# klory/vqa-attention-networks

Measured on AMD Instinct MI355X. Metric: QA-pairs/sec fwd+bwd, MFB-baseline batch 512, higher is better.
Workload: dtype f32

## Files before the change

### include/vqa_fusion.h

```cpp
#ifndef VQA_FUSION_H
#define VQA_FUSION_H

#include <stddef.h>
#include <stdint.h>

#ifdef __cplusplus
extern "C" {
#endif

#define VQF_OK 0
#define VQF_E_BADARG (-1)
#define VQF_E_ALIGN (-2)
#define VQF_E_UNSUPPORTED (-3)
#define VQF_E_WORKSPACE (-4)
#define VQF_E_TIMEOUT (-5)

#define VQF_POOL_K 5

#define VQF_GEMM_RELU 1
#define VQF_GEMM_ACCUM 2
#define VQF_GEMM_OUT_BF16 4

int vqf_abi_version(void);
const char* vqf_build_info(void);
// ... 4 lines not shown
#define VQF_OPT_GEMM_BF16_LOOP 3
#define VQF_OPT_GEMM_F32_BIG 4
#define VQF_OPT_GEMM_BF16_BIG 5
#define VQF_OPT_GEMM_F32_WAVE 6
#define VQF_OPT_FUSE_COAL 7
#define VQF_OPT_FUSE_LS 8
#define VQF_OPT_FUSE_LS_BWD 9
#define VQF_OPT_GEMM_CU_LIMIT 10
#define VQF_OPT_GEMM_F32_EDGE 11
#define VQF_OPT_GEMM_F32_ROUNDS 12
#define VQF_OPT_GEMM_SPLITK_FUSED 13
#define VQF_OPT_GEMM_F32_STREAMK 14
#define VQF_OPT_GEMM_SPLITK_ORDER 15
#define VQF_OPT_GEMM_F32_SAMPLE 16
#define VQF_OPT_GEMM_F32_N80 17
#define VQF_OPT_COUNT 18
int vqf_set_option(int option, int value, int* previous);
int vqf_get_option(int option, int* value);
const char* vqf_option_env_name(int option);

#define VQF_STAT_GEMM_F32_TILE128 0
#define VQF_STAT_GEMM_F32_BIG 1
#define VQF_STAT_GEMM_F32_WAVE 2
#define VQF_STAT_GEMM_BF16_TILE128 3
#define VQF_STAT_GEMM_BF16_BIG 4
#define VQF_STAT_GEMM_F32_SAMPLE 5
#define VQF_STAT_GEMM_F32_N80 6
#define VQF_STAT_COUNT 7
int vqf_stat_get(int stat, long long* value);

size_t vqf_gemm_f32_ws_bytes(int ta, int tb, int M, int N, int K);
int vqf_gemm_f32(int ta, int tb, int M, int N, int K,
                 const float* A, int lda, const float* B, int ldb,
                 float* C, int ldc, const float* bias, int flags,
                 void* ws, size_t ws_bytes, void* stream);

int vqf_gemm_f32_rowscale(int ta, int tb, int M, int N, int K, const float* A, int lda, const float* B, int ldb,
                          float* C, int ldc, const float* bias, int flags, const float* rowscale, int rows_per_scale,
                          void* stream);

int vqf_gemm_f32_big_rows(int ta, int tb, int M, int N, int K);
int vqf_gemm_f32_sample_supported(int NS, int L, int N, int K);
int vqf_gemm_f32_sample(int tb, int NS, int L, int N, int K, const float* A, int lda, const float* B, int ldb, float* C, int ldc,
// ... 261 lines not shown
int vqf_lstm_seq_supported(int B, int H);
size_t vqf_lstm_seq_ws_bytes(int B, int H);
#define VQF_LSTM_BF16 1
int vqf_lstm_seq_fwd(const float* xw, const float* w_hh, int S, int B, int H,
                     float* hs, float* cs, float* gates, int flags, void* ws, size_t ws_bytes, void* stream);
int vqf_lstm_seq_bwd(const float* dhs, const float* gates, const float* cs, const float* w_hh,
                     int S, int B, int H, float* dgates, float* dc_carry, int flags, void* ws, size_t ws_bytes,
                     void* stream);

int vqf_lstm_cell_fwd(float* gates, const float* c_prev, int B, int H, float* c_out, float* h_out, void* stream);
int vqf_lstm_step_supported(int B, int H);
int vqf_lstm_step_fwd(const float* h_prev, const float* w_hh, float* gates, const float* c_prev, int B, int H,
                      float* c_out, float* h_out, void* stream);
int vqf_lstm_cell_bwd(const float* dhs_t, const float* dh_carry, const float* gates, const float* c_t,
                      const float* c_prev, int first, int B, int H, float* dc_carry, float* dG, void* stream);

int vqf_embed_tanh_fwd(const float* W, const long long* ids, int T, int V, int E, float* out, void* stream);
int vqf_embed_tanh_bwd(const float* dout, const float* out, const long long* ids, int T, int V, int E, float* dW,
                       void* stream);
int vqf_embed_fwd(const float* W, const long long* ids, int T, int V, int E, float* out, void* stream);
int vqf_embed_bwd(const float* dout, const long long* ids, int T, int V, int E, float* dW, void* stream);
int vqf_embed_dropout_fwd(const float* W, const long long* ids, int T, int V, int E, const uint8_t* keep, uint64_t seed, float p_drop,
                          float* out, void* stream);
int vqf_embed_dropout_bwd(const float* dout, const long long* ids, int T, int V, int E, const uint8_t* keep, uint64_t seed, float p_drop,
                          float* dW, void* stream);
int vqf_embed_tanh_fwd_tm(const float* W, const long long* ids, int N, int Tq, int V, int E, float* out, void* stream);
int vqf_embed_tanh_bwd_tm(const float* dout, const float* out, const long long* ids, int N, int Tq, int V, int E, float* dW,
                          void* stream);

int vqf_feat_transpose(const float* src, int N, int D, int L, int out_bf16, void* dst, void* stream);
// ... 46 lines not shown
```

### vqa-attention-networks_amd/csrc/common.h

```cpp
#pragma once
#include <hip/hip_runtime.h>
#include <stdint.h>
#include "../../include/vqa_fusion.h"

typedef float f32x4 __attribute__((ext_vector_type(4)));
typedef float f32x16 __attribute__((ext_vector_type(16)));
typedef unsigned int u32x4 __attribute__((ext_vector_type(4)));

enum VqfKernelId {
  KID_GEMM_A0B0 = 0,
  KID_GEMM_A0B1,
  KID_GEMM_A1B0,
  KID_GEMM_A1B1,
  KID_SPLITK_REDUCE,
  KID_COLSUM,
  KID_GROUP_REDUCE,
  KID_RELU_BWD,
  KID_ATT_LOGITS_FWD,
  KID_ATT_LOGITS_BWD,
  KID_GLIMPSE_FWD,
  KID_GLIMPSE_BWD,
  KID_MFB_FUSE_FWD,
  KID_L2_GROUP_NORM,
  KID_SCALE_ROWS,
// ... 28 lines not shown
  KID_HIE_SLABSUM,
  KID_HIE_AFF,
  KID_PHRASE_FWD,
  KID_PHRASE_BWD,
  KID_HIE_AFF_LEVELS,
  KID_GUIDED_FWD,
  KID_GUIDED_BWD,
  KID_CE_LOSS_PRED,
  KID_ANSWER_MATCH,
  KID_TOPK_ROWS,
  KID_GLIMPSE_DFEAT_GROUPED,
  KID_ROW_BLOCK_GATHER,
  KID_ROW_BLOCK_GROUP_SUM,
  KID_MFB_FUSE_BWD_IMAGE,
  KID_ZERO_COLS,
  KID_COUNT
};

extern int g_vqf_prof_on;
extern int g_vqf_opt[VQF_OPT_COUNT];
static inline int vqf_opt(int id, int dflt) { const int v = g_vqf_opt[id]; return v < 0 ? dflt : v; }
extern long long g_vqf_stat[VQF_STAT_COUNT];
static inline void vqf_stat_bump(int id) { __atomic_fetch_add(&g_vqf_stat[id], 1LL, __ATOMIC_RELAXED); }
bool vqf_prof_begin(int id, hipStream_t s);
void vqf_prof_end(int id, hipStream_t s);
void vqf_prof_dims(int d0, int d1, int d2);

#define VQF_LAUNCH(id, kern, grid, block, shmem, stream, ...)                      \
  do {                                                                             \
    (void)hipGetLastError();     \
// ... 11 lines not shown
int* vqf_splitk_counters(int tiles);

int vqf_gemm_bf16_big_try(int ta, int tb, int M, int N, int K, const void* A, int lda, const void* B, int ldb, float* C,
                          int ldc, const float* bias, int flags, const float* rowscale, int rps, void* ws, size_t ws_bytes,
                          hipStream_t s, int* rc);
size_t vqf_gemm_bf16_big_ws_bytes(int ta, int tb, int M, int N, int K);
int vqf_gemm_f32_big_try(int ta, int tb, int M, int N, int K, const float* A, int lda, const float* B, int ldb, float* C,
                         int ldc, const float* bias, int flags, const float* rowscale, int rps, void* ws, size_t ws_bytes,
                         hipStream_t s, int* rc, int* rows_done);
int vqf_gemm_f32_big_rows_impl(int ta, int tb, int M, int N, int K, int flags, size_t ws_bytes);
size_t vqf_gemm_f32_big_ws_bytes(int ta, int tb, int M, int N, int K);
int vqf_gemm_f32_n80_try(int M, int N, int K, const float* A, int lda, const float* B, int ldb, float* C, int ldc,
                         const float* bias, int flags, hipStream_t s, int* rc);
int vqf_lstm_step16_try(const float* h_prev, const float* w_hh, float* gates, const float* c_prev, int B, int H, float* c_out,
                        float* h_out, hipStream_t s, int* rc);
int vqf_gemm_f32_wave_try(int ta, int tb, int M, int N, int K, const float* A, int lda, const float* B, int ldb, float* C,
                          int ldc, const float* bias, int flags, hipStream_t s, int* rc);

static inline int vqf_last_error() {
  hipError_t e = hipGetLastError();
  return e == hipSuccess ? VQF_OK : (int)e;
}

static inline bool aligned16(const void* p) { return (((uintptr_t)p) & 15) == 0; }

struct VqfDynLdsFlags { int bytes[64]; };
static inline int vqf_set_dyn_lds(const void* fn, int bytes, VqfDynLdsFlags& f) {
  int dev = 0;
  (void)hipGetDevice(&dev);
  const bool tracked = dev >= 0 && dev < 64;
// ... 187 lines not shown
```

### vqa-attention-networks_amd/csrc/gemm_f32_n80.hip

```cpp
#include "common.h"

namespace {

typedef const float __attribute__((address_space(1))) gfloat;

constexpr int TM = 128, TN = 80, TK = 32, NT = 512, NSLOT = 4;
constexpr int A_BYTES = TM * TK * 4;
constexpr int b_bytes(int ntc) { return 16 * ntc * TK * 4; }
constexpr int slot_bytes(int ntc) { return A_BYTES + b_bytes(ntc); }

struct N80Args {
  const float* A; const float* B; float* C; const float* bias;
  int M, N, K, lda, ldb, ldc, flags, tiles_m, tiles;
  const float* c_prev; float* c_out; float* h_out; int H;
};

__device__ __forceinline__ float sigm_f(float x) { return 1.0f / (1.0f + expf(-x)); }

__device__ __forceinline__ int swz(int rho) {
  const int i = (rho >> 1) & 7;
  return i ^ (((i + 2) & 4) >> 1);
}

__device__ __forceinline__ void wait_own(int later, bool two) {
// ... 136 lines not shown
#pragma unroll
  for (int t = 0; t < NTC; ++t) {
    const int col = n0 + 16 * t + c;
    if (col < g.N) {
      const float bv = g.bias ? g.bias[col] : 0.f;
#pragma unroll
      for (int j = 0; j < 4; ++j) {
        const int row = m0 + 16 * wave + 4 * kq + j;
        if (row < g.M) {
          float v = acc[t][j] + bv;
          if (relu) v = fmaxf(v, 0.f);
          g.C[(long long)row * g.ldc + col] = v;
        }
      }
    }
  }
}

}

int vqf_gemm_f32_n80_try(int M, int N, int K, const float* A, int lda, const float* B, int ldb, float* C, int ldc,
                         const float* bias, int flags, hipStream_t s, int* rc) {
  if (vqf_opt(VQF_OPT_GEMM_F32_N80, 1) == 0) return 0;
  if ((flags & ~VQF_GEMM_RELU) || (K % 128) || K < 512 || !aligned16(A) || !aligned16(B) || (lda % 4) || (ldb % 4)) return 0;
  const int tiles_m = (M + TM - 1) / TM, tiles_n = (N + TN - 1) / TN;
  const long long tiles = (long long)tiles_m * tiles_n;
  const int cus = vqf_cu_count() > 0 ? vqf_cu_count() : 256;
  if (tiles > cus || tiles * 10 < (long long)cus * 8 || M > 1024) return 0;
  if (vqf_opt(VQF_OPT_GEMM_CU_LIMIT, 0) >= 8) return 0;
  N80Args g;
// ... 18 lines not shown
  const int cus = vqf_cu_count() > 0 ? vqf_cu_count() : 256;
  if (tiles > cus || tiles * 10 < (long long)cus * 8) return 0;
  N80Args g = {};
  g.A = h_prev; g.B = w_hh; g.C = gates; g.M = B; g.N = 4 * H; g.K = H; g.lda = H; g.ldb = H; g.ldc = 4 * H;
  g.tiles_m = tiles_m; g.tiles = (int)tiles;
  g.c_prev = c_prev; g.c_out = c_out; g.h_out = h_out; g.H = H;
  const int nwg = ((int)tiles + 7) & ~7;
  vqf_prof_dims(B, 4 * H, H);
  vqf_stat_bump(VQF_STAT_GEMM_F32_N80);
  static VqfDynLdsFlags attr = {};
  if (int e = vqf_set_dyn_lds(reinterpret_cast<const void*>(&gemm_f32_n80_kernel<4, true>), NSLOT * slot_bytes(4), attr)) { *rc = e; return 1; }
  VQF_LAUNCH(KID_LSTM_CELL_FWD, (gemm_f32_n80_kernel<4, true>), dim3(nwg), dim3(NT), NSLOT * slot_bytes(4), s, g);
  *rc = vqf_last_error();
  return 1;
}
```

### vqa-attention-networks_amd/csrc/gemm_f32_wave.hip

```cpp
#include "common.h"
#include <stdlib.h>

namespace {

typedef const float __attribute__((address_space(1))) gfloat;
typedef float f32x2 __attribute__((ext_vector_type(2)));

constexpr int WTM = 32, WTN = 64, TK = 16, NSLOT = 6, NT = 256;
constexpr int A_BYTES = WTM * TK * 4, B_BYTES = WTN * TK * 4, SLOT_BYTES = A_BYTES + B_BYTES;
constexpr int WAVE_LDS = NSLOT * SLOT_BYTES;
constexpr int SMEM_WAVE = 4 * WAVE_LDS;
constexpr int NGA = A_BYTES / 1024, NGB = B_BYTES / 1024, NGL = NGA + NGB;

struct WaveArgs {
  const float* A;
  const float* B;
  float* C;
  const float* bias;
  int M, N, K, lda, ldb, ldc, flags;
  int tiles_m, tiles_n, kpart;
  const float* c_prev;
  float* c_out;
  float* h_out;
  int H;
};

__device__ __forceinline__ int swz(int r) { return (r >> 2) & 3; }

template <bool TB>
__device__ __forceinline__ void init_src(gfloat* (&q)[NGL], const WaveArgs& g, int m0, int n0, int k0, int lane) {
#pragma unroll
  for (int i = 0; i < NGA; ++i) {
    const int row = 16 * i + (lane >> 2);
    const int chunk = (lane & 3) ^ swz(row);
    q[i] = (gfloat*)(g.A + (long long)min(m0 + row, g.M - 1) * g.lda + k0 + chunk * 4);
  }
#pragma unroll
  for (int i = 0; i < NGB; ++i) {
    if (!TB) {
// ... 61 lines not shown

__device__ __forceinline__ void c_prefetch(const WaveArgs& g, int m0, int n0, int lane, bool vec, f32x2 (&cold)[16]) {
  const int cm = lane & 31, h = lane >> 5, col = n0 + 2 * cm;
#pragma unroll
  for (int e = 0; e < 16; ++e) {
    cold[e] = f32x2{0.f, 0.f};
    const int row = m0 + (e & 3) + 8 * (e >> 2) + 4 * h;
    if ((g.flags & VQF_GEMM_ACCUM) && row < g.M && col < g.N) {
      const float* pc = g.C + (long long)row * g.ldc + col;
      if (vec && col + 1 < g.N) cold[e] = *reinterpret_cast<const f32x2*>(pc);
      else { cold[e][0] = pc[0]; if (col + 1 < g.N) cold[e][1] = pc[1]; }
    }
  }
}

template <bool TB, int WK>
__global__ void __launch_bounds__(NT, 1) gemm_f32_wave_kernel(const WaveArgs g) {
  extern __shared__ __attribute__((aligned(16))) char smem[];
  const int tid = threadIdx.x, lane = tid & 63;
  const int wave = __builtin_amdgcn_readfirstlane(tid >> 6);
  const int nwg = gridDim.x, bid = blockIdx.x;
  const int q8 = nwg >> 3, r8 = nwg & 7, xcd = bid & 7;
  const int wg = (xcd < r8 ? xcd * (q8 + 1) : r8 * (q8 + 1) + (xcd - r8) * q8) + (bid >> 3);
  const int t = (WK == 1) ? 4 * wg + wave : wg;
  const int ntiles = g.tiles_m * g.tiles_n;
  const bool live = t < ntiles;
  const int tm = live ? t % g.tiles_m : 0, tn = live ? t / g.tiles_m : 0;
  const int m0 = tm * WTM, n0 = tn * WTN;
  const int k0 = (WK == 1) ? 0 : wave * g.kpart;
  const int S = live ? g.kpart / TK : 0;
  char* my = smem + wave * WAVE_LDS;

  f32x16 acc[2];
#pragma unroll
  for (int j = 0; j < 2; ++j)
#pragma unroll
    for (int e = 0; e < 16; ++e) acc[j][e] = 0.f;

  gfloat* q[NGL];
  init_src<TB>(q, g, m0, n0, k0, lane);
#pragma unroll
  for (int p = 0; p < NSLOT - 1; ++p)
    if (p < S) stage<TB>(q, g, my + p * SLOT_BYTES);
  const bool vec = ((g.ldc & 1) == 0) && ((reinterpret_cast<uintptr_t>(g.C) & 7) == 0);
  f32x2 cold[16];
  if (WK == 1 && live) c_prefetch(g, m0, n0, lane, vec, cold);
  Frag<TB> fa[2], fb[2];
  int slot = 0;
  auto half = [&](int s, Frag<TB> (&cur)[2], Frag<TB> (&nxt)[2]) {
    const bool more = s + 1 < S, refill = s + NSLOT - 1 < S;
    if (more) wait_copies(min(NSLOT - 3, S - 2 - s));
    const char* nx = my + (slot + 1 == NSLOT ? 0 : slot + 1) * SLOT_BYTES;
    char* rf = my + ((slot == 0) ? NSLOT - 1 : slot - 1) * SLOT_BYTES;
    typedef __attribute__((address_space(3))) char lds_char;
#pragma unroll
    for (int n = 0; n < 16; ++n) {
      const int ks = n >> 3, e = (n >> 1) & 3, j = n & 1;
      acc[j] = __builtin_amdgcn_mfma_f32_32x32x2f32(cur[ks].a[e], cur[ks].b(j, e), acc[j], 0, 0, 0);
      if (n == 0 && more) nxt[0].load(nx, 0, lane);
      if (n == 2 && more) nxt[1].load(nx, 1, lane);
      if (n >= 4 && n < 4 + NGL && refill) {
// ... 19 lines not shown
    half(s, fa, fb);
    if (s + 1 < S) half(s + 1, fb, fa);
  }

  const int cm = lane & 31, h = lane >> 5;
  if (WK == 1) {
    if (!live) return;
    const int col = n0 + 2 * cm;
    const float b0 = (g.bias && col < g.N) ? g.bias[col] : 0.f;
    const float b1 = (g.bias && col + 1 < g.N) ? g.bias[col + 1] : 0.f;
#pragma unroll
    for (int e = 0; e < 16; ++e)
      put2(g, m0 + (e & 3) + 8 * (e >> 2) + 4 * h, col, acc[0][e], acc[1][e], b0, b1, vec, cold[e][0], cold[e][1]);
  } else {
    asm volatile("s_waitcnt vmcnt(0)" ::: "memory");
    f32x2* mine = reinterpret_cast<f32x2*>(my);
#pragma unroll
    for (int e = 0; e < 16; ++e) mine[e * 64 + lane] = f32x2{acc[0][e], acc[1][e]};
    __syncthreads();
    if (!live) return;
    const int col = n0 + 2 * cm;
    const float b0 = (g.bias && col < g.N) ? g.bias[col] : 0.f;
    const float b1 = (g.bias && col + 1 < g.N) ? g.bias[col + 1] : 0.f;
#pragma unroll
    for (int qd = 0; qd < 4; ++qd) {
      const int e = wave + 4 * qd;
      f32x2 v = reinterpret_cast<const f32x2*>(smem)[e * 64 + lane];
#pragma unroll
      for (int w = 1; w < 4; ++w) {
        const f32x2 p = reinterpret_cast<const f32x2*>(smem + w * WAVE_LDS)[e * 64 + lane];
        v[0] += p[0]; v[1] += p[1];
      }
      float c0 = 0.f, c1 = 0.f;
      const int row = m0 + (e & 3) + 8 * (e >> 2) + 4 * h;
      if ((g.flags & VQF_GEMM_ACCUM) && row < g.M && col < g.N) {
        c0 = g.C[(long long)row * g.ldc + col];
        if (col + 1 < g.N) c1 = g.C[(long long)row * g.ldc + col + 1];
      }
      put2(g, row, col, v[0], v[1], b0, b1, vec, c0, c1);
    }
  }
}

constexpr int NGS = NGA + 1;

__device__ __forceinline__ void wait_copies3(int later) {
  switch (later < 0 ? 0 : later) {
    case 0:  asm volatile("s_waitcnt vmcnt(0)" ::: "memory"); break;
    case 1:  asm volatile("s_waitcnt vmcnt(3)" ::: "memory"); break;
// ... 245 lines not shown
    pc[2 * H] = a1;
    const float f_act = __shfl_xor(a0, 16, 64), o_act = __shfl_xor(a1, 16, 64);
    if (lo) {
      const float c = f_act * cpv[e] + a0 * a1;
      g.c_out[(long long)row * H + u0 + cm] = c;
      g.h_out[(long long)row * H + u0 + cm] = o_act * tanhf(c);
    }
  }
}

int launch_lstm_fwd(const WaveArgs& g, int nwg, hipStream_t s) {
  static VqfDynLdsFlags attr = {};
  constexpr int SMEM_SHB = 6 * (4 * A_BYTES + B_BYTES);
  if (int e = vqf_set_dyn_lds(reinterpret_cast<const void*>(&gemm_f32_lstm_fwd_kernel), SMEM_SHB, attr)) return e;
  VQF_LAUNCH(KID_LSTM_CELL_FWD, gemm_f32_lstm_fwd_kernel, dim3(nwg), dim3(NT), SMEM_SHB, s, g);
  return vqf_last_error();
}

template <bool TB, int WK>
int launch(const WaveArgs& g, int nwg, hipStream_t s) {
  static VqfDynLdsFlags attr = {};
  if (int e = vqf_set_dyn_lds(reinterpret_cast<const void*>(&gemm_f32_wave_kernel<TB, WK>), SMEM_WAVE, attr)) return e;
  VQF_LAUNCH(KID_GEMM_A0B0 + (TB ? 1 : 0), (gemm_f32_wave_kernel<TB, WK>), dim3(nwg), dim3(NT), SMEM_WAVE, s, g);
  return vqf_last_error();
}

}

int vqf_gemm_f32_wave_try(int ta, int tb, int M, int N, int K, const float* A, int lda, const float* B, int ldb, float* C,
                          int ldc, const float* bias, int flags, hipStream_t s, int* rc) {
// ... 38 lines not shown
  {
    int rc = VQF_OK;
    if (vqf_lstm_step16_try(h_prev, w_hh, gates, c_prev, B, H, c_out, h_out, (hipStream_t)stream, &rc)) return rc;
  }
  WaveArgs g = {};
  g.A = h_prev; g.B = w_hh; g.C = gates; g.bias = nullptr;
  g.M = B; g.N = 4 * H; g.K = H; g.lda = H; g.ldb = H; g.ldc = 4 * H; g.flags = VQF_GEMM_ACCUM;
  g.tiles_m = B / WTM;
  g.tiles_n = H / 16;
  g.kpart = H;
  g.c_prev = c_prev; g.c_out = c_out; g.h_out = h_out; g.H = H;
  vqf_prof_dims(B, 4 * H, H);
  vqf_stat_bump(VQF_STAT_GEMM_F32_WAVE);
  return launch_lstm_fwd(g, g.tiles_m * g.tiles_n / 4, (hipStream_t)stream);
}
```

### vqa-attention-networks_amd/csrc/prof.hip

```cpp
#include "common.h"
#include <mutex>
#include <stdlib.h>
#include <vector>

int g_vqf_prof_on = 0;
int g_vqf_opt[VQF_OPT_COUNT];
long long g_vqf_stat[VQF_STAT_COUNT] = {};

namespace {
const char* const kOptEnv[VQF_OPT_COUNT] = {
    "VQF_GEMM_F32_PERSIST", "VQF_GEMM_BF16_PERSIST", "VQF_GEMM_F32_LOOP", "VQF_GEMM_BF16_LOOP", "VQF_GEMM_F32_BIG",
    "VQF_GEMM_BF16_BIG", "VQF_GEMM_F32_WAVE", "VQF_FUSE_COAL", "VQF_FUSE_LS", "VQF_FUSE_LS_BWD", "VQF_GEMM_CU_LIMIT",
    "VQF_GEMM_F32_EDGE", "VQF_GEMM_F32_ROUNDS", "VQF_GEMM_SPLITK_FUSED", "VQF_GEMM_F32_STREAMK", "VQF_GEMM_SPLITK_ORDER", "VQF_GEMM_F32_SAMPLE", "VQF_GEMM_F32_N80"};
const char* const kOptEnvOld[VQF_OPT_COUNT] = {
    nullptr, nullptr, "VQF_GEMM_F32_PP", "VQF_GEMM_BF16_PP", nullptr, nullptr, nullptr, nullptr, nullptr, nullptr, nullptr,
    nullptr, nullptr, nullptr, nullptr, nullptr, nullptr};
struct OptInit {
  OptInit() {
    for (int i = 0; i < VQF_OPT_COUNT; ++i) {
      const char* e = getenv(kOptEnv[i]);
      if (!e && kOptEnvOld[i]) e = getenv(kOptEnvOld[i]);
      g_vqf_opt[i] = (e && ((e[0] >= '0' && e[0] <= '9') || e[0] == '-')) ? atoi(e) : -1;
    }
  }
} g_opt_init;
}

namespace {
// ... 5 lines not shown
thread_local int t_dims[3] = {0, 0, 0};
long long g_min_mnk = 0;

const char* const kNames[KID_COUNT] = {
    "gemm_f32_a0b0(fwd)", "gemm_f32_a0b1(dgrad)", "gemm_f32_a1b0", "gemm_f32_a1b1(wgrad)",
    "splitk_reduce", "colsum", "group_reduce", "relu_bwd",
    "att_logits_fwd", "att_logits_bwd", "glimpse_pool_fwd", "glimpse_pool_bwd",
    "mfb_fuse_fwd", "l2_group_norm", "scale_rows", "rowdot", "l2_norm_bwd_coef", "mfb_fuse_bwd",
    "dropout", "tanh_dropout_fwd", "tanh_dropout_bwd", "softmax_rows_fwd", "softmax_rows_bwd",
    "gemm_bf16", "cast_f32_bf16",
    "lstm_seq_fwd(all steps)", "lstm_seq_bwd(all steps)",
    "ce_loss", "kldiv_loss", "adam_step", "feat_transpose",
    "lstm_cell_fwd", "lstm_cell_bwd", "embed_tanh_fwd", "embed_tanh_bwd", "hbm_copy", "hbm_read_sweep", "multi_add", "multi_copy", "hie_hv_fwd", "hie_head_bwd", "hie_rank_add", "hie_rank_left", "hie_slab_sum", "hie_affinity",
    "phrase_ngram_fwd", "phrase_ngram_bwd", "hie_affinity_levels", "guided_logits_fwd", "guided_logits_bwd",
    "ce_loss_pred", "answer_match_rows", "topk_rows", "glimpse_dfeat_grouped", "row_block_gather", "row_block_group_sum",
    "mfb_fuse_bwd_image", "zero_cols_len"};

hipEvent_t get_event() {
  std::lock_guard<std::mutex> lk(g_mu);
  if (!g_free.empty()) { hipEvent_t e = g_free.back(); g_free.pop_back(); return e; }
  hipEvent_t e = nullptr;
  (void)hipEventCreate(&e);
  return e;
}
}

bool vqf_prof_begin(int id, hipStream_t s) {
  if (g_min_mnk > 0) {
    const bool gemm = (id >= KID_GEMM_A0B0 && id <= KID_GEMM_A1B1) || id == KID_GEMM_BF16;
    if (!gemm || (long long)t_dims[0] * t_dims[1] * t_dims[2] < g_min_mnk) return false;
  }
// ... 70 lines not shown
```

### vqa-attention-networks_amd/host/functions.py

```python
import torch

from . import ops


def _c(t):
    return t if t.is_contiguous() else t.contiguous()


def _w2d(w):
    return _c(w.reshape(w.shape[0], -1))


def _bf16_ok(*dims):
    return all(d % 8 == 0 for d in dims)


class EmbedTanhFn(torch.autograd.Function):

    @staticmethod
    def forward(ctx, ids, weight, tanh=True, time_major=False, lens=None):
        ids = ids.contiguous()
        out = ops.embed_tanh_fwd(_c(weight), ids, tanh, time_major, lens=lens)
        ctx.save_for_backward(ids, out if tanh else None)
        ctx.V, ctx.tm, ctx.lens = weight.shape[0], bool(time_major), lens
# ... 1005 lines not shown
                    ops.gemm(hs[t - 1], whh, out=gates[t], accumulate=True)
            ops.lstm_cell_fwd(gates[t], cs[t - 1] if t else None, cs[t], hs[t])
        ctx.save_for_backward(x, w_ih, w_hh, hs, cs, gates, xb, wb)
        ctx.has_bias = b_ih is not None
        return hs

    @staticmethod
    def backward(ctx, dhs):
        x, w_ih, w_hh, hs, cs, gates, xb, wb = ctx.saved_tensors
        T, B, I = x.shape
        H = w_hh.shape[1]
        dhs = _c(dhs)
        whh = ops.cast_bf16(_c(w_hh)) if ctx.bf16 else _c(w_hh)
        dG = torch.empty_like(gates)
        dc = torch.empty((B, H), dtype=torch.float32, device=x.device)
        dh = None
        for t in range(T - 1, -1, -1):
            ops.lstm_cell_bwd(dhs[t], dh, gates[t], cs[t], cs[t - 1] if t else None, t == T - 1, dc, dG[t])
            if t > 0:
                dh = ops.gemm_bf16(ops.cast_bf16(dG[t]), whh, tb=True) if ctx.bf16 else ops.gemm(dG[t], whh, tb=True)
        dG2 = dG.view(T * B, 4 * H)
        if ctx.bf16_proj:
            dGb = ops.cast_bf16(dG2)
            dx, dw_ih = _lstm_in_proj_bwd(dGb, xb, wb, I, ctx.needs_input_grad[0])
            dx = dx.view(T, B, I) if dx is not None else None
        else:
            dx = ops.gemm(dG2, _c(w_ih), tb=True).view(T, B, I) if ctx.needs_input_grad[0] else None
            dw_ih = ops.gemm(dG2, x.view(T * B, I), ta=True, tb=True)
        if T > 1 and ctx.bf16_proj and B % 8 == 0:
            dw_hh = ops.gemm_bf16(dGb[B:], ops.cast_bf16(hs[:-1].reshape((T - 1) * B, H)), ta=True, tb=True)
        elif T > 1:
            dw_hh = ops.gemm(dG[1:].reshape((T - 1) * B, 4 * H), hs[:-1].reshape((T - 1) * B, H), ta=True, tb=True)
        else:
            dw_hh = torch.zeros_like(w_hh)
        db = ops.colsum(dG2) if ctx.has_bias else None
# ... 42 lines not shown
```

### vqa-attention-networks_amd/host/lib.py

```python
import ctypes
import os
import subprocess
import threading

_HERE = os.path.dirname(os.path.abspath(__file__))
PKG_DIR = os.path.dirname(_HERE)
CSRC_DIR = os.path.join(PKG_DIR, "csrc")
LIB_PATH = os.path.join(PKG_DIR, "libvqa_fusion.so")
if os.environ.get("VQF_LIB"):
    LIB_PATH = os.path.abspath(os.environ["VQF_LIB"])
HEADER_PATH = os.path.join(os.path.dirname(PKG_DIR), "include", "vqa_fusion.h")

ABI_VERSION = 7

_lock = threading.Lock()
_lib = None

c_f = ctypes.c_void_p
c_i = ctypes.c_int
c_sz = ctypes.c_size_t
c_u64 = ctypes.c_uint64
c_p = ctypes.c_void_p

SIGNATURES = {
# ... 134 lines not shown
                                      c_i, c_i, c_i, c_i, c_f, c_f, c_f, c_p, c_sz, c_p]),
    "vqf_mfb_fuse_fwd_grouped_packed": (c_i, [c_f, c_f, c_f, c_p, c_p, c_p, c_u64, ctypes.c_float, c_i, c_i, c_i, c_i, c_i, c_f, c_f,
                                              c_p]),
    "vqf_mfb_fuse_bwd_grouped_packed": (c_i, [c_f, c_f, c_f, c_f, c_f, c_f, c_f, c_f, c_p, c_p, c_p, c_p, c_p, c_u64, ctypes.c_float,
                                              c_i, c_i, c_i, c_i, c_i, c_f, c_f, c_f, c_p, c_sz, c_p]),
    "vqf_glimpse_pool_fwd_packed": (c_i, [c_f, c_f, c_p, c_p, c_i, c_i, c_i, c_i, c_i, c_i, c_i, c_f, c_f, c_p]),
    "vqf_glimpse_pool_bwd_packed": (c_i, [c_f, c_f, c_f, c_f, c_p, c_p, c_i, c_i, c_i, c_i, c_i, c_i, c_i, c_f, c_p]),
    "vqf_lstm_seq_supported": (c_i, [c_i, c_i]),
    "vqf_lstm_seq_ws_bytes": (c_sz, [c_i, c_i]),
    "vqf_lstm_seq_fwd": (c_i, [c_f, c_f, c_i, c_i, c_i, c_f, c_f, c_f, c_i, c_p, c_sz, c_p]),
    "vqf_lstm_seq_bwd": (c_i, [c_f, c_f, c_f, c_f, c_i, c_i, c_i, c_f, c_f, c_i, c_p, c_sz, c_p]),
    "vqf_lstm_cell_fwd": (c_i, [c_f, c_f, c_i, c_i, c_f, c_f, c_p]),
    "vqf_lstm_step_supported": (c_i, [c_i, c_i]),
    "vqf_lstm_step_fwd": (c_i, [c_f, c_f, c_f, c_f, c_i, c_i, c_f, c_f, c_p]),
    "vqf_lstm_cell_bwd": (c_i, [c_f, c_f, c_f, c_f, c_f, c_i, c_i, c_i, c_f, c_f, c_p]),
    "vqf_embed_tanh_fwd": (c_i, [c_f, c_p, c_i, c_i, c_i, c_f, c_p]),
    "vqf_embed_tanh_bwd": (c_i, [c_f, c_f, c_p, c_i, c_i, c_i, c_f, c_p]),
    "vqf_embed_fwd": (c_i, [c_f, c_p, c_i, c_i, c_i, c_f, c_p]),
    "vqf_embed_bwd": (c_i, [c_f, c_p, c_i, c_i, c_i, c_f, c_p]),
    "vqf_embed_dropout_fwd": (c_i, [c_f, c_p, c_i, c_i, c_i, c_p, c_u64, ctypes.c_float, c_f, c_p]),
    "vqf_embed_dropout_bwd": (c_i, [c_f, c_p, c_i, c_i, c_i, c_p, c_u64, ctypes.c_float, c_f, c_p]),
    "vqf_embed_tanh_fwd_tm": (c_i, [c_f, c_p, c_i, c_i, c_i, c_i, c_f, c_p]),
    "vqf_embed_tanh_bwd_tm": (c_i, [c_f, c_f, c_p, c_i, c_i, c_i, c_i, c_f, c_p]),
    "vqf_feat_transpose": (c_i, [c_f, c_i, c_i, c_i, c_i, c_p, c_p]),
    "vqf_loss_ws_bytes": (c_sz, [c_i, c_i]),
    "vqf_ce_loss": (c_i, [c_f, c_p, c_i, c_i, c_f, c_f, c_p, c_sz, c_p]),
    "vqf_kldiv_loss": (c_i, [c_f, c_f, c_i, c_i, c_f, c_f, c_p, c_sz, c_p]),
    "vqf_ce_loss_pred": (c_i, [c_f, c_p, c_i, c_i, c_f, c_f, c_p, c_p, c_p, c_f, c_i, c_p, c_sz, c_p]),
    "vqf_answer_match_rows": (c_i, [c_f, c_f, c_i, c_i, c_p, c_p, c_f, c_p, c_p, c_f, c_p, c_f, c_i, c_p, c_sz, c_p]),
    "vqf_topk_rows_supported": (c_i, [c_i, c_i]),
# ... 79 lines not shown
```

### vqa-attention-networks_amd/host/ops.py

```python
import ctypes
import math
import torch

from . import lib as _l

GEMM_RELU = 1
GEMM_ACCUM = 2
POOL_K = 5


def _lib():
    return _l.load()


def _stream():
    return ctypes.c_void_p(torch.cuda.current_stream().cuda_stream)


def _ptr(t):
    return ctypes.c_void_p(t.data_ptr()) if t is not None else ctypes.c_void_p(0)


def _chk(*ts):
    for t in ts:
# ... 22 lines not shown
            self.bufs[key] = b
        return b


_ws = _Workspace()
SPLITK_WS_BYTES = 192 << 20


def workspace(device, nbytes):
    return _ws.get(device, nbytes)


OPTIONS = {"gemm_f32_persist": 0, "gemm_bf16_persist": 1, "gemm_f32_loop": 2, "gemm_bf16_loop": 3, "gemm_f32_big": 4,
           "gemm_bf16_big": 5, "gemm_f32_wave": 6, "fuse_coal": 7, "fuse_ls": 8, "fuse_ls_bwd": 9, "gemm_cu_limit": 10,
           "gemm_f32_edge": 11, "gemm_f32_rounds": 12, "gemm_splitk_fused": 13, "gemm_f32_streamk": 14,
           "gemm_splitk_order": 15, "gemm_f32_sample": 16, "gemm_f32_n80": 17}


def set_option(name, value):
    prev = ctypes.c_int(0)
    _l.check(_lib().vqf_set_option(OPTIONS[name], -1 if value is None else int(value), ctypes.byref(prev)),
             "vqf_set_option(%s)" % name)
    return prev.value


def get_option(name):
    v = ctypes.c_int(0)
    _l.check(_lib().vqf_get_option(OPTIONS[name], ctypes.byref(v)), "vqf_get_option(%s)" % name)
    return v.value


STATS = {"gemm_f32_tile128": 0, "gemm_f32_big": 1, "gemm_f32_wave": 2, "gemm_bf16_tile128": 3, "gemm_bf16_big": 4,
         "gemm_f32_sample": 5, "gemm_f32_n80": 6}


def stat(name):
    v = ctypes.c_longlong(0)
    _l.check(_lib().vqf_stat_get(STATS[name], ctypes.byref(v)), "vqf_stat_get(%s)" % name)
    return v.value


class options:

    def __init__(self, **kw):
        self.kw, self.prev = kw, {}

    def __enter__(self):
        for k, v in self.kw.items():
# ... 1245 lines not shown

def lstm_step_fwd(h_prev, w_hh, gates, c_prev, c_out, h_out):
    _chk(h_prev, w_hh, gates, c_prev, c_out, h_out)
    B, H4 = gates.shape
    _l.check(_lib().vqf_lstm_step_fwd(_ptr(h_prev), _ptr(w_hh), _ptr(gates), _ptr(c_prev), B, H4 // 4, _ptr(c_out), _ptr(h_out),
                                      _stream()), "vqf_lstm_step_fwd")


def lstm_cell_bwd(dhs_t, dh_carry, gates, c_t, c_prev, first, dc_carry, dG):
    _chk(dhs_t, dh_carry, gates, c_t, c_prev, dc_carry, dG)
    B, H = dhs_t.shape
    _l.check(_lib().vqf_lstm_cell_bwd(_ptr(dhs_t), _ptr(dh_carry), _ptr(gates), _ptr(c_t), _ptr(c_prev), int(bool(first)),
                                      B, H, _ptr(dc_carry), _ptr(dG), _stream()), "vqf_lstm_cell_bwd")


def _chk_ids(ids):
    if not ids.is_cuda or ids.dtype != torch.int64 or not ids.is_contiguous():
        raise _l.VqfError("contiguous int64 GPU token ids expected")


def embed_tanh_fwd(weight, ids, tanh=True, time_major=False, lens=None):
    _chk(weight)
    _chk_ids(ids)
    V, E = weight.shape
    T = ids.numel()
    if lens is not None:
        if not tanh or time_major or ids.dim() != 2:
            raise _l.VqfError("embed_tanh_fwd: lens goes with (N, Tq) ids, tanh and sample-major rows")
        N, Tq = ids.shape
        _chk_lens(lens, N, "embed_tanh_fwd")
# ... 264 lines not shown
```

Measured before the change: 12760.

## Fuse LSTM backward recurrent GEMM with the previous step's cell backward

The f32 LSTM backward loop used to run a separate cell-backward kernel and a dG·W_hh GEMM on every timestep. It now launches one fused kernel per step: the wave GEMM epilogue computes dh and applies the cell-backward gate math in place, writing dG_prev and dc_carry directly. This removes one launch per step and the dh round trip through memory, but the epilogue carries extra loads and register pressure. An alternative split-K tile kernel with atomic tile counters is added but stays off by default.

```diff
diff --git a/include/vqa_fusion.h b/include/vqa_fusion.h
--- a/include/vqa_fusion.h
+++ b/include/vqa_fusion.h
@@ -42,7 +42,8 @@
 #define VQF_OPT_GEMM_SPLITK_ORDER 15
 #define VQF_OPT_GEMM_F32_SAMPLE 16
 #define VQF_OPT_GEMM_F32_N80 17
-#define VQF_OPT_COUNT 18
+#define VQF_OPT_LSTM_STEP_BWD 18
+#define VQF_OPT_COUNT 19
 int vqf_set_option(int option, int value, int* previous);
 int vqf_get_option(int option, int* value);
 const char* vqf_option_env_name(int option);
@@ -54,7 +55,9 @@
 #define VQF_STAT_GEMM_BF16_BIG 4
 #define VQF_STAT_GEMM_F32_SAMPLE 5
 #define VQF_STAT_GEMM_F32_N80 6
-#define VQF_STAT_COUNT 7
+#define VQF_STAT_LSTM_STEP_BWD_WAVE 7
+#define VQF_STAT_LSTM_STEP_BWD_TILE 8
+#define VQF_STAT_COUNT 9
 int vqf_stat_get(int stat, long long* value);
 
 size_t vqf_gemm_f32_ws_bytes(int ta, int tb, int M, int N, int K);
@@ -346,6 +349,10 @@
                       float* c_out, float* h_out, void* stream);
 int vqf_lstm_cell_bwd(const float* dhs_t, const float* dh_carry, const float* gates, const float* c_t,
                       const float* c_prev, int first, int B, int H, float* dc_carry, float* dG, void* stream);
+int vqf_lstm_step_bwd_supported(int B, int H);
+int vqf_lstm_step_bwd(const float* dG_t, const float* w_hh, const float* dhs_prev, const float* gates_prev,
+                      const float* c_prev, const float* c_prev2, int B, int H, float* dc_carry, float* dG_prev,
+                      float* dh_out, void* stream);
 
 int vqf_embed_tanh_fwd(const float* W, const long long* ids, int T, int V, int E, float* out, void* stream);
 int vqf_embed_tanh_bwd(const float* dout, const float* out, const long long* ids, int T, int V, int E, float* dW,
diff --git a/vqa-attention-networks_amd/csrc/common.h b/vqa-attention-networks_amd/csrc/common.h
--- a/vqa-attention-networks_amd/csrc/common.h
+++ b/vqa-attention-networks_amd/csrc/common.h
@@ -66,6 +66,7 @@
   KID_ROW_BLOCK_GROUP_SUM,
   KID_MFB_FUSE_BWD_IMAGE,
   KID_ZERO_COLS,
+  KID_LSTM_STEP_BWD,
   KID_COUNT
 };
 
@@ -107,6 +108,9 @@
                          const float* bias, int flags, hipStream_t s, int* rc);
 int vqf_lstm_step16_try(const float* h_prev, const float* w_hh, float* gates, const float* c_prev, int B, int H, float* c_out,
                         float* h_out, hipStream_t s, int* rc);
+int vqf_lstm_step_bwd_tile_try(const float* dG_t, const float* w_hh, const float* dhs_prev, const float* gates_prev,
+                               const float* c_prev, const float* c_prev2, int B, int H, float* dc_carry, float* dG_prev,
+                               float* dh_out, int force, hipStream_t s, int* rc);
 int vqf_gemm_f32_wave_try(int ta, int tb, int M, int N, int K, const float* A, int lda, const float* B, int ldb, float* C,
                           int ldc, const float* bias, int flags, hipStream_t s, int* rc);
 
diff --git a/vqa-attention-networks_amd/csrc/gemm_f32_n80.hip b/vqa-attention-networks_amd/csrc/gemm_f32_n80.hip
--- a/vqa-attention-networks_amd/csrc/gemm_f32_n80.hip
+++ b/vqa-attention-networks_amd/csrc/gemm_f32_n80.hip
@@ -174,6 +174,151 @@
         }
       }
     }
+  }
+}
+
+struct StepBwdArgs {
+  const float* A; const float* W; const float* dhs; const float* gates; const float* c1; const float* c2;
+  float* dc; float* dG; float* dh_out; int* cnt;
+  int B, H, tiles_m, items;
+};
+
+__global__ void __launch_bounds__(NT, 1) lstm_step_bwd_tile_kernel(const StepBwdArgs g) {
+  constexpr int SLOT_BYTES = slot_bytes(4), NFR = 10;
+  extern __shared__ __attribute__((aligned(16))) char smem[];
+  typedef __attribute__((address_space(3))) char lds_char;
+  const int per = (gridDim.x + 7) >> 3;
+  const int lin = (blockIdx.x & 7) * per + (blockIdx.x >> 3);
+  if (lin >= g.items) return;
+  const int z = lin & 3, tile = lin >> 2;
+  const int tn = tile / g.tiles_m, tm = tile - tn * g.tiles_m;
+  const int m0 = tm * TM, n0 = tn * 64, H = g.H;
+  const int tid = threadIdx.x, lane = tid & 63;
+  const int wave = __builtin_amdgcn_readfirstlane(tid >> 6);
+  const int c = lane & 15, kq = lane >> 4;
+  const int S = H / TK;
+
+  gfloat* qa[2];
+#pragma unroll
+  for (int i = 0; i < 2; ++i) {
+    const int ra = 16 * wave + 8 * i + (lane >> 3);
+    qa[i] = (gfloat*)(g.A + (long long)(m0 + ra) * (4 * H) + (long long)z * H + 4 * ((lane & 7) ^ swz(ra)));
+  }
+  gfloat* qb = (gfloat*)(g.W + ((long long)z * H + 4 * wave + (lane >> 4)) * H + n0 + 4 * (lane & 15));
+  auto issue_piece = [&](int s, int slot, int p) {
+    lds_char* da = (lds_char*)(smem + slot * SLOT_BYTES + wave * 2048);
+    lds_char* db = (lds_char*)(smem + slot * SLOT_BYTES + A_BYTES + wave * 1024);
+    if (p == 0)      __builtin_amdgcn_global_load_lds(qa[0] + (long long)s * TK, da, 16, 0, 0);
+    else if (p == 1) __builtin_amdgcn_global_load_lds(qa[1] + (long long)s * TK, da + 1024, 16, 0, 0);
+    else if (p == 2) __builtin_amdgcn_global_load_lds(qb + (long long)s * TK * H, db, 16, 0, 0);
+  };
+
+  f32x4 acc[4];
+#pragma unroll
+  for (int t = 0; t < 4; ++t) acc[t] = f32x4{0.f, 0.f, 0.f, 0.f};
+
+  struct Frag { f32x4 a[2], b[2][4]; };
+  auto read_frag = [&](int slot, Frag& f, int i) {
+    const char* sa = smem + slot * SLOT_BYTES;
+    if (i < 2) {
+      const int ra = 16 * wave + c;
+      f.a[i] = *reinterpret_cast<const f32x4*>(sa + ra * 128 + (((2 * kq + i) ^ swz(ra)) << 4));
+    } else {
+      const int u = (i - 2) >> 2, j = (i - 2) & 3;
+      f.b[u][j] = *reinterpret_cast<const f32x4*>(sa + A_BYTES + (8 * kq + 4 * u + j) * 256 + (c << 4));
+    }
+  };
+  auto step = [&](int s, int q, const Frag& cur, Frag& nxt) {
+    const bool more = s + 1 < S, copy = s + NSLOT < S;
+#pragma unroll
+    for (int grp = 0; grp < 8; ++grp) {
+      const int u = grp >> 2, j = grp & 3;
+#pragma unroll
+      for (int t = 0; t < 4; ++t) acc[t] = __builtin_amdgcn_mfma_f32_16x16x4f32(cur.a[u][j], cur.b[u][j][t], acc[t], 0, 0, 0);
+      if (grp < 3) { if (copy) issue_piece(s + NSLOT, q, grp); }
+      if (more && 2 * grp < NFR) { read_frag((q + 1) % NSLOT, nxt, 2 * grp); read_frag((q + 1) % NSLOT, nxt, 2 * grp + 1); }
+      __builtin_amdgcn_sched_barrier(0);
+    }
+  };
+#pragma unroll
+  for (int p = 0; p < NSLOT; ++p) {
+#pragma unroll
+    for (int i = 0; i < 3; ++i) issue_piece(p, p, i);
+  }
+  Frag fr[2];
+  wait_own(NSLOT - 1, false);
+  __builtin_amdgcn_s_barrier();
+#pragma unroll
+  for (int i = 0; i < NFR; ++i) read_frag(0, fr[0], i);
+  for (int s0 = 0; s0 < S; s0 += NSLOT) {
+#pragma unroll
+    for (int q = 0; q < NSLOT; ++q) {
+      const int s = s0 + q;
+      if (s < S) {
+        if (s + 1 < S) wait_own(min(NSLOT - 2, S - 2 - s), false);
+        __builtin_amdgcn_s_waitcnt(0xC07F);
+        __builtin_amdgcn_s_barrier();
+        step(s, q, fr[q & 1], fr[(q + 1) & 1]);
+      }
+    }
+  }
+
+  const int col = n0 + 4 * c;
+#pragma unroll
+  for (int j = 0; j < 4; ++j) {
+    const long long row = m0 + 16 * wave + 4 * kq + j;
+    *reinterpret_cast<f32x4*>(g.dG + row * 4 * H + (long long)z * H + col) = f32x4{acc[0][j], acc[1][j], acc[2][j], acc[3][j]};
+  }
+  asm volatile("s_waitcnt vmcnt(0)" ::: "memory");
+  __syncthreads();
+  int* scratch = reinterpret_cast<int*>(smem);
+  if (tid == 0) {
+    __builtin_amdgcn_fence(__ATOMIC_RELEASE, "agent");
+    asm volatile("s_waitcnt vmcnt(0)" ::: "memory");
+    const int ticket = __hip_atomic_fetch_add(g.cnt + tile, 1, __ATOMIC_RELAXED, __HIP_MEMORY_SCOPE_AGENT);
+    *reinterpret_cast<volatile int*>(scratch) = ticket;
+  }
+  __syncthreads();
+  const int ticket = *reinterpret_cast<volatile int*>(scratch);
+  if (ticket != 3) return;
+  if (tid == 0) {
+    __builtin_amdgcn_fence(__ATOMIC_ACQUIRE, "agent");
+    asm volatile("s_waitcnt vmcnt(0)" ::: "memory");
+    __hip_atomic_store(g.cnt + tile, 0, __ATOMIC_RELAXED, __HIP_MEMORY_SCOPE_AGENT);
+  }
+  __syncthreads();
+#pragma unroll
+  for (int j = 0; j < 4; ++j) {
+    const long long row = m0 + 16 * wave + 4 * kq + j;
+    const long long bh = row * H + col;
+    float* d = g.dG + row * 4 * H + col;
+    f32x4 p[4];
+#pragma unroll
+    for (int k = 0; k < 4; ++k) p[k] = *reinterpret_cast<const f32x4*>(d + (long long)k * H);
+    const float* gp = g.gates + row * 4 * H + col;
+    const f32x4 gi = *reinterpret_cast<const f32x4*>(gp), gf = *reinterpret_cast<const f32x4*>(gp + H);
+    const f32x4 gg = *reinterpret_cast<const f32x4*>(gp + 2 * H), go = *reinterpret_cast<const f32x4*>(gp + 3 * H);
+    const f32x4 cc = *reinterpret_cast<const f32x4*>(g.c1 + bh);
+    f32x4 cp = {0.f, 0.f, 0.f, 0.f};
+    if (g.c2) cp = *reinterpret_cast<const f32x4*>(g.c2 + bh);
+    const f32x4 dcc = *reinterpret_cast<const f32x4*>(g.dc + bh);
+    f32x4 dh = *reinterpret_cast<const f32x4*>(g.dhs + bh);
+    dh += ((p[0] + p[1]) + p[2]) + p[3];
+    f32x4 d0, d1, d2, d3, dco;
+#pragma unroll
+    for (int e = 0; e < 4; ++e) {
+      const float tc = tanhf(cc[e]);
+      const float dc = dcc[e] + dh[e] * go[e] * (1.0f - tc * tc);
+      d0[e] = dc * gg[e] * gi[e] * (1.0f - gi[e]);
+      d1[e] = dc * cp[e] * gf[e] * (1.0f - gf[e]);
+      d2[e] = dc * gi[e] * (1.0f - gg[e] * gg[e]);
+      d3[e] = dh[e] * tc * go[e] * (1.0f - go[e]);
+      dco[e] = dc * gf[e];
+    }
+    *reinterpret_cast<f32x4*>(d) = d0; *reinterpret_cast<f32x4*>(d + H) = d1;
+    *reinterpret_cast<f32x4*>(d + 2 * H) = d2; *reinterpret_cast<f32x4*>(d + 3 * H) = d3;
+    *reinterpret_cast<f32x4*>(g.dc + bh) = dco;
+    if (g.dh_out) *reinterpret_cast<f32x4*>(g.dh_out + bh) = dh;
   }
 }
 
@@ -222,3 +367,29 @@
   *rc = vqf_last_error();
   return 1;
 }
+
+int vqf_lstm_step_bwd_tile_try(const float* dG_t, const float* w_hh, const float* dhs_prev, const float* gates_prev,
+                               const float* c_prev, const float* c_prev2, int B, int H, float* dc_carry, float* dG_prev,
+                               float* dh_out, int force, hipStream_t s, int* rc) {
+  if (vqf_opt(VQF_OPT_GEMM_CU_LIMIT, 0) >= 8) return 0;
+  if ((B % TM) || (H % 64) || H < 256) return 0;
+  const int tiles_m = B / TM, tiles = tiles_m * (H / 64);
+  const long long items = 4LL * tiles;
+  const int cus = vqf_cu_count() > 0 ? vqf_cu_count() : 256;
+  if (!force && (items > cus || items * 10 < (long long)cus * 8)) return 0;
+  int* cnt = vqf_splitk_counters(tiles);
+  if (!cnt) return 0;
+  StepBwdArgs g = {};
+  g.A = dG_t; g.W = w_hh; g.dhs = dhs_prev; g.gates = gates_prev; g.c1 = c_prev; g.c2 = c_prev2;
+  g.dc = dc_carry; g.dG = dG_prev; g.dh_out = dh_out; g.cnt = cnt;
+  g.B = B; g.H = H; g.tiles_m = tiles_m; g.items = (int)items;
+  const int nwg = ((int)items + 7) & ~7;
+  vqf_prof_dims(B, H, 4 * H);
+  vqf_stat_bump(VQF_STAT_LSTM_STEP_BWD_TILE);
+  static VqfDynLdsFlags attr = {};
+  if (int e = vqf_set_dyn_lds(reinterpret_cast<const void*>(&lstm_step_bwd_tile_kernel), NSLOT * slot_bytes(4), attr)) { *rc = e; return 1; }
+  VQF_LAUNCH(KID_LSTM_STEP_BWD, lstm_step_bwd_tile_kernel, dim3(nwg), dim3(NT), NSLOT * slot_bytes(4), s, g);
+  *rc = vqf_last_error();
+  if (*rc != VQF_OK) vqf_splitk_counters_clear(cnt, tiles, s);
+  return 1;
+}
diff --git a/vqa-attention-networks_amd/csrc/gemm_f32_wave.hip b/vqa-attention-networks_amd/csrc/gemm_f32_wave.hip
--- a/vqa-attention-networks_amd/csrc/gemm_f32_wave.hip
+++ b/vqa-attention-networks_amd/csrc/gemm_f32_wave.hip
@@ -23,6 +23,13 @@
   float* c_out;
   float* h_out;
   int H;
+  const float* dhs_prev;
+  const float* gates_prev;
+  const float* cb_t;
+  const float* cb_prev;
+  float* dc_carry;
+  float* dG_prev;
+  float* dh_out;
 };
 
 __device__ __forceinline__ int swz(int r) { return (r >> 2) & 3; }
@@ -114,8 +121,9 @@
   }
 }
 
-template <bool TB, int WK>
+template <bool TB, int WK, bool CELLB = false>
 __global__ void __launch_bounds__(NT, 1) gemm_f32_wave_kernel(const WaveArgs g) {
+  static_assert(!CELLB || (TB && WK == 4), "the LSTM backward step is the K-major, four-K-range form");
   extern __shared__ __attribute__((aligned(16))) char smem[];
   const int tid = threadIdx.x, lane = tid & 63;
   const int wave = __builtin_amdgcn_readfirstlane(tid >> 6);
@@ -145,6 +153,25 @@
   const bool vec = ((g.ldc & 1) == 0) && ((reinterpret_cast<uintptr_t>(g.C) & 7) == 0);
   f32x2 cold[16];
   if (WK == 1 && live) c_prefetch(g, m0, n0, lane, vec, cold);
+  f32x2 x_dhs[4], x_g[4][4], x_c[4], x_cp[4], x_dc[4];
+  auto cell_fetch = [&]() {
+    const int cm = lane & 31, h = lane >> 5;
+    const int colc = n0 + 2 * cm;
+#pragma unroll
+    for (int qd = 0; qd < 4; ++qd) {
+      const int row = m0 + wave + 8 * qd + 4 * h;
+      const bool in = live && row < g.M && colc < g.N;
+      const long long bh = (long long)row * g.H + colc;
+      const f32x2 z2 = {0.f, 0.f};
+      x_dhs[qd] = in ? *reinterpret_cast<const f32x2*>(g.dhs_prev + bh) : z2;
+#pragma unroll
+      for (int k = 0; k < 4; ++k)
+        x_g[qd][k] = in ? *reinterpret_cast<const f32x2*>(g.gates_prev + (long long)row * 4 * g.H + k * g.H + colc) : z2;
+      x_c[qd] = in ? *reinterpret_cast<const f32x2*>(g.cb_t + bh) : z2;
+      x_cp[qd] = (in && g.cb_prev) ? *reinterpret_cast<const f32x2*>(g.cb_prev + bh) : z2;
+      x_dc[qd] = in ? *reinterpret_cast<const f32x2*>(g.dc_carry + bh) : z2;
+    }
+  };
   Frag<TB> fa[2], fb[2];
   int slot = 0;
   auto half = [&](int s, Frag<TB> (&cur)[2], Frag<TB> (&nxt)[2]) {
@@ -194,6 +221,7 @@
       put2(g, m0 + (e & 3) + 8 * (e >> 2) + 4 * h, col, acc[0][e], acc[1][e], b0, b1, vec, cold[e][0], cold[e][1]);
   } else {
     asm volatile("s_waitcnt vmcnt(0)" ::: "memory");
+    if (CELLB) cell_fetch();
     f32x2* mine = reinterpret_cast<f32x2*>(my);
 #pragma unroll
     for (int e = 0; e < 16; ++e) mine[e * 64 + lane] = f32x2{acc[0][e], acc[1][e]};
@@ -213,6 +241,33 @@
       }
       float c0 = 0.f, c1 = 0.f;
       const int row = m0 + (e & 3) + 8 * (e >> 2) + 4 * h;
+      if (CELLB) {
+        if (row >= g.M || col >= g.N) continue;
+        const long long bh = (long long)row * g.H + col;
+        f32x2 dh2, d0, d1, d2, d3, dco;
+        v[0] += b0; v[1] += b1;
+#pragma unroll
+        for (int j = 0; j < 2; ++j) {
+          const float gi = x_g[qd][0][j], gf = x_g[qd][1][j], gg = x_g[qd][2][j], go = x_g[qd][3][j];
+          const float dh = x_dhs[qd][j] + v[j];
+          const float tc = tanhf(x_c[qd][j]);
+          const float dc = x_dc[qd][j] + dh * go * (1.0f - tc * tc);
+          d0[j] = dc * gg * gi * (1.0f - gi);
+          d1[j] = dc * x_cp[qd][j] * gf * (1.0f - gf);
+          d2[j] = dc * gi * (1.0f - gg * gg);
+          d3[j] = dh * tc * go * (1.0f - go);
+          dco[j] = dc * gf;
+          dh2[j] = dh;
+        }
+        float* d = g.dG_prev + (long long)row * 4 * g.H + col;
+        *reinterpret_cast<f32x2*>(d) = d0;
+        *reinterpret_cast<f32x2*>(d + g.H) = d1;
+        *reinterpret_cast<f32x2*>(d + 2 * g.H) = d2;
+        *reinterpret_cast<f32x2*>(d + 3 * g.H) = d3;
+        *reinterpret_cast<f32x2*>(g.dc_carry + bh) = dco;
+        if (g.dh_out) *reinterpret_cast<f32x2*>(g.dh_out + bh) = dh2;
+        continue;
+      }
       if ((g.flags & VQF_GEMM_ACCUM) && row < g.M && col < g.N) {
         c0 = g.C[(long long)row * g.ldc + col];
         if (col + 1 < g.N) c1 = g.C[(long long)row * g.ldc + col + 1];
@@ -488,6 +543,13 @@
   constexpr int SMEM_SHB = 6 * (4 * A_BYTES + B_BYTES);
   if (int e = vqf_set_dyn_lds(reinterpret_cast<const void*>(&gemm_f32_lstm_fwd_kernel), SMEM_SHB, attr)) return e;
   VQF_LAUNCH(KID_LSTM_CELL_FWD, gemm_f32_lstm_fwd_kernel, dim3(nwg), dim3(NT), SMEM_SHB, s, g);
+  return vqf_last_error();
+}
+
+int launch_lstm_bwd(const WaveArgs& g, int nwg, hipStream_t s) {
+  static VqfDynLdsFlags attr = {};
+  if (int e = vqf_set_dyn_lds(reinterpret_cast<const void*>(&gemm_f32_wave_kernel<true, 4, true>), SMEM_WAVE, attr)) return e;
+  VQF_LAUNCH(KID_LSTM_STEP_BWD, (gemm_f32_wave_kernel<true, 4, true>), dim3(nwg), dim3(NT), SMEM_WAVE, s, g);
   return vqf_last_error();
 }
 
@@ -556,3 +618,37 @@
   vqf_stat_bump(VQF_STAT_GEMM_F32_WAVE);
   return launch_lstm_fwd(g, g.tiles_m * g.tiles_n / 4, (hipStream_t)stream);
 }
+
+#define VQF_LSTM_STEP_BWD_TILE_DEFAULT 0
+extern "C" int vqf_lstm_step_bwd_supported(int B, int H) {
+  return B > 0 && H >= 256 && (B % 128) == 0 && (H % 16) == 0 && vqf_opt(VQF_OPT_GEMM_F32_WAVE, 2) != 0 &&
+         vqf_opt(VQF_OPT_LSTM_STEP_BWD, 1) != 0;
+}
+extern "C" int vqf_lstm_step_bwd(const float* dG_t, const float* w_hh, const float* dhs_prev, const float* gates_prev,
+                                 const float* c_prev, const float* c_prev2, int B, int H, float* dc_carry, float* dG_prev,
+                                 float* dh_out, void* stream) {
+  if (!dG_t || !w_hh || !dhs_prev || !gates_prev || !c_prev || !dc_carry || !dG_prev || B <= 0 || H <= 0) return VQF_E_BADARG;
+  if (!vqf_lstm_step_bwd_supported(B, H)) return VQF_E_UNSUPPORTED;
+  if (!aligned16(dG_t) || !aligned16(w_hh) || !aligned16(dhs_prev) || !aligned16(gates_prev) || !aligned16(c_prev) ||
+      !aligned16(dc_carry) || !aligned16(dG_prev) || (c_prev2 && !aligned16(c_prev2)) || (dh_out && !aligned16(dh_out)))
+    return VQF_E_ALIGN;
+  const int form = vqf_opt(VQF_OPT_LSTM_STEP_BWD, 1);
+  if (form == 2 || (form == 1 && VQF_LSTM_STEP_BWD_TILE_DEFAULT)) {
+    int rc = VQF_OK;
+    if (vqf_lstm_step_bwd_tile_try(dG_t, w_hh, dhs_prev, gates_prev, c_prev, c_prev2, B, H, dc_carry, dG_prev, dh_out, form == 2,
+                                   (hipStream_t)stream, &rc))
+      return rc;
+  }
+  WaveArgs g = {};
+  g.A = dG_t; g.B = w_hh; g.C = nullptr; g.bias = nullptr;
+  g.M = B; g.N = H; g.K = 4 * H; g.lda = 4 * H; g.ldb = H; g.ldc = H; g.flags = 0;
+  g.tiles_m = B / WTM;
+  g.tiles_n = (H + WTN - 1) / WTN;
+  g.kpart = H;
+  g.H = H;
+  g.dhs_prev = dhs_prev; g.gates_prev = gates_prev; g.cb_t = c_prev; g.cb_prev = c_prev2;
+  g.dc_carry = dc_carry; g.dG_prev = dG_prev; g.dh_out = dh_out;
+  vqf_prof_dims(B, H, 4 * H);
+  vqf_stat_bump(VQF_STAT_LSTM_STEP_BWD_WAVE);
+  return launch_lstm_bwd(g, g.tiles_m * g.tiles_n, (hipStream_t)stream);
+}
diff --git a/vqa-attention-networks_amd/csrc/prof.hip b/vqa-attention-networks_amd/csrc/prof.hip
--- a/vqa-attention-networks_amd/csrc/prof.hip
+++ b/vqa-attention-networks_amd/csrc/prof.hip
@@ -11,7 +11,8 @@
 const char* const kOptEnv[VQF_OPT_COUNT] = {
     "VQF_GEMM_F32_PERSIST", "VQF_GEMM_BF16_PERSIST", "VQF_GEMM_F32_LOOP", "VQF_GEMM_BF16_LOOP", "VQF_GEMM_F32_BIG",
     "VQF_GEMM_BF16_BIG", "VQF_GEMM_F32_WAVE", "VQF_FUSE_COAL", "VQF_FUSE_LS", "VQF_FUSE_LS_BWD", "VQF_GEMM_CU_LIMIT",
-    "VQF_GEMM_F32_EDGE", "VQF_GEMM_F32_ROUNDS", "VQF_GEMM_SPLITK_FUSED", "VQF_GEMM_F32_STREAMK", "VQF_GEMM_SPLITK_ORDER", "VQF_GEMM_F32_SAMPLE", "VQF_GEMM_F32_N80"};
+    "VQF_GEMM_F32_EDGE", "VQF_GEMM_F32_ROUNDS", "VQF_GEMM_SPLITK_FUSED", "VQF_GEMM_F32_STREAMK", "VQF_GEMM_SPLITK_ORDER", "VQF_GEMM_F32_SAMPLE", "VQF_GEMM_F32_N80",
+    "VQF_LSTM_STEP_BWD"};
 const char* const kOptEnvOld[VQF_OPT_COUNT] = {
     nullptr, nullptr, "VQF_GEMM_F32_PP", "VQF_GEMM_BF16_PP", nullptr, nullptr, nullptr, nullptr, nullptr, nullptr, nullptr,
     nullptr, nullptr, nullptr, nullptr, nullptr, nullptr};
@@ -47,7 +48,7 @@
     "lstm_cell_fwd", "lstm_cell_bwd", "embed_tanh_fwd", "embed_tanh_bwd", "hbm_copy", "hbm_read_sweep", "multi_add", "multi_copy", "hie_hv_fwd", "hie_head_bwd", "hie_rank_add", "hie_rank_left", "hie_slab_sum", "hie_affinity",
     "phrase_ngram_fwd", "phrase_ngram_bwd", "hie_affinity_levels", "guided_logits_fwd", "guided_logits_bwd",
     "ce_loss_pred", "answer_match_rows", "topk_rows", "glimpse_dfeat_grouped", "row_block_gather", "row_block_group_sum",
-    "mfb_fuse_bwd_image", "zero_cols_len"};
+    "mfb_fuse_bwd_image", "zero_cols_len", "lstm_step_bwd"};
 
 hipEvent_t get_event() {
   std::lock_guard<std::mutex> lk(g_mu);
diff --git a/vqa-attention-networks_amd/host/functions.py b/vqa-attention-networks_amd/host/functions.py
--- a/vqa-attention-networks_amd/host/functions.py
+++ b/vqa-attention-networks_amd/host/functions.py
@@ -1043,11 +1043,16 @@
         whh = ops.cast_bf16(_c(w_hh)) if ctx.bf16 else _c(w_hh)
         dG = torch.empty_like(gates)
         dc = torch.empty((B, H), dtype=torch.float32, device=x.device)
-        dh = None
-        for t in range(T - 1, -1, -1):
-            ops.lstm_cell_bwd(dhs[t], dh, gates[t], cs[t], cs[t - 1] if t else None, t == T - 1, dc, dG[t])
-            if t > 0:
-                dh = ops.gemm_bf16(ops.cast_bf16(dG[t]), whh, tb=True) if ctx.bf16 else ops.gemm(dG[t], whh, tb=True)
+        if not ctx.bf16 and T > 1 and ops.lstm_step_bwd_supported(B, H):
+            ops.lstm_cell_bwd(dhs[T - 1], None, gates[T - 1], cs[T - 1], cs[T - 2], True, dc, dG[T - 1])
+            for t in range(T - 1, 0, -1):
+                ops.lstm_step_bwd(dG[t], whh, dhs[t - 1], gates[t - 1], cs[t - 1], cs[t - 2] if t > 1 else None, dc, dG[t - 1])
+        else:
+            dh = None
+            for t in range(T - 1, -1, -1):
+                ops.lstm_cell_bwd(dhs[t], dh, gates[t], cs[t], cs[t - 1] if t else None, t == T - 1, dc, dG[t])
+                if t > 0:
+                    dh = ops.gemm_bf16(ops.cast_bf16(dG[t]), whh, tb=True) if ctx.bf16 else ops.gemm(dG[t], whh, tb=True)
         dG2 = dG.view(T * B, 4 * H)
         if ctx.bf16_proj:
             dGb = ops.cast_bf16(dG2)
diff --git a/vqa-attention-networks_amd/host/lib.py b/vqa-attention-networks_amd/host/lib.py
--- a/vqa-attention-networks_amd/host/lib.py
+++ b/vqa-attention-networks_amd/host/lib.py
@@ -172,6 +172,8 @@
     "vqf_lstm_step_supported": (c_i, [c_i, c_i]),
     "vqf_lstm_step_fwd": (c_i, [c_f, c_f, c_f, c_f, c_i, c_i, c_f, c_f, c_p]),
     "vqf_lstm_cell_bwd": (c_i, [c_f, c_f, c_f, c_f, c_f, c_i, c_i, c_i, c_f, c_f, c_p]),
+    "vqf_lstm_step_bwd_supported": (c_i, [c_i, c_i]),
+    "vqf_lstm_step_bwd": (c_i, [c_f, c_f, c_f, c_f, c_f, c_f, c_i, c_i, c_f, c_f, c_f, c_p]),
     "vqf_embed_tanh_fwd": (c_i, [c_f, c_p, c_i, c_i, c_i, c_f, c_p]),
     "vqf_embed_tanh_bwd": (c_i, [c_f, c_f, c_p, c_i, c_i, c_i, c_f, c_p]),
     "vqf_embed_fwd": (c_i, [c_f, c_p, c_i, c_i, c_i, c_f, c_p]),
diff --git a/vqa-attention-networks_amd/host/ops.py b/vqa-attention-networks_amd/host/ops.py
--- a/vqa-attention-networks_amd/host/ops.py
+++ b/vqa-attention-networks_amd/host/ops.py
@@ -60,7 +60,7 @@
 OPTIONS = {"gemm_f32_persist": 0, "gemm_bf16_persist": 1, "gemm_f32_loop": 2, "gemm_bf16_loop": 3, "gemm_f32_big": 4,
            "gemm_bf16_big": 5, "gemm_f32_wave": 6, "fuse_coal": 7, "fuse_ls": 8, "fuse_ls_bwd": 9, "gemm_cu_limit": 10,
            "gemm_f32_edge": 11, "gemm_f32_rounds": 12, "gemm_splitk_fused": 13, "gemm_f32_streamk": 14,
-           "gemm_splitk_order": 15, "gemm_f32_sample": 16, "gemm_f32_n80": 17}
+           "gemm_splitk_order": 15, "gemm_f32_sample": 16, "gemm_f32_n80": 17, "lstm_step_bwd": 18}
 
 
 def set_option(name, value):
@@ -77,7 +77,7 @@
 
 
 STATS = {"gemm_f32_tile128": 0, "gemm_f32_big": 1, "gemm_f32_wave": 2, "gemm_bf16_tile128": 3, "gemm_bf16_big": 4,
-         "gemm_f32_sample": 5, "gemm_f32_n80": 6}
+         "gemm_f32_sample": 5, "gemm_f32_n80": 6, "lstm_step_bwd_wave": 7, "lstm_step_bwd_tile": 8}
 
 
 def stat(name):
@@ -1353,6 +1353,17 @@
                                       B, H, _ptr(dc_carry), _ptr(dG), _stream()), "vqf_lstm_cell_bwd")
 
 
+def lstm_step_bwd_supported(B, H):
+    return bool(_lib().vqf_lstm_step_bwd_supported(int(B), int(H)))
+
+
+def lstm_step_bwd(dG_t, w_hh, dhs_prev, gates_prev, c_prev, c_prev2, dc_carry, dG_prev, dh_out=None):
+    _chk(dG_t, w_hh, dhs_prev, gates_prev, c_prev, c_prev2, dc_carry, dG_prev, dh_out)
+    B, H = dhs_prev.shape
+    _l.check(_lib().vqf_lstm_step_bwd(_ptr(dG_t), _ptr(w_hh), _ptr(dhs_prev), _ptr(gates_prev), _ptr(c_prev), _ptr(c_prev2), B, H,
+                                      _ptr(dc_carry), _ptr(dG_prev), _ptr(dh_out), _stream()), "vqf_lstm_step_bwd")
+
+
 def _chk_ids(ids):
     if not ids.is_cuda or ids.dtype != torch.int64 or not ids.is_contiguous():
         raise _l.VqfError("contiguous int64 GPU token ids expected")
```

Result: no change. 12800, median of 6 (+0.3%).
